# lh3/bfc

Hardware: AMD Instinct MI355X
Metric: M k-mers/s counted (bloom+htab) on 150 bp reads (higher is better)
Workload: dtype u64

## Files before the change

bfc_amd/csrc/bfcg_bloom3.hip:

```cpp
#include <hip/hip_runtime.h>
#include <stdint.h>
#include <stdlib.h>
#include "kmer_dev.h"
#include "bfcg_internal.h"
#include "bfcg_dev.h"

using namespace bfcg;

#define B3_UND 0x40000000u
#define B3_SEEN16 0x8000u
#define B3_COLD_NR 8
#define B3_WALK_U 4
template <int BT, int PF, bool COLD>
__global__ __launch_bounds__(BT, PF <= 2 ? 8 : 6) void k_bloom3(KParams P, BloomArgs A)
{
	extern __shared__ __attribute__((aligned(16))) unsigned char smem[];
	__shared__ uint32_t s_list_n, s_ovf, s_pool_off, s_emit_n, s_fs_used, s_wb_n, s_pad3[2];
	const uint32_t f = blockIdx.x;
	const bool ho_log = A.ho_stride != 0;
	if (batch_poisoned(A)) { if (ho_log && threadIdx.x == 0) A.ho_mark[f] = A.ho_cur[f]; return; }
	uint32_t rs, n;
	region_list(A, f, rs, n);
	if (n == 0) { if (threadIdx.x == 0) { if (ho_log) A.ho_mark[f] = A.ho_cur[f]; else if (A.agg_cnt) A.agg_cnt[f] = 0; } return; }
	uint32_t ho_cur0 = 0;
	unsigned long long *ho_base;
	if (ho_log) {
		ho_cur0 = A.ho_cur[f];
		if (ho_cur0 + n > A.ho_stride) {
			if (threadIdx.x == 0) { atomicAdd(&A.stats[(size_t)(f & (ST_SLOTS - 1)) * ST_N + ST_ERR_POOL], 1ULL); A.ho_mark[f] = ho_cur0; }
			return;
		}
		ho_base = A.ho + (uint64_t)f * A.ho_stride + ho_cur0;
	} else ho_base = reinterpret_cast<unsigned long long *>(A.stream_out) + rs;
	A.stats += (size_t)(f & (ST_SLOTS - 1)) * ST_N;
	const uint32_t region_dw = 16u << P.R;
	unsigned char *sp = smem;
	unsigned int *region = reinterpret_cast<unsigned int *>(sp); sp += (size_t)region_dw * 4;
	const uint32_t nblk = 1u << P.R;
	unsigned int *bcnt = reinterpret_cast<unsigned int *>(sp), *boff = bcnt + nblk;
	if (COLD) sp += (size_t)(2 * nblk + 4) * 4;
	unsigned int *fs = reinterpret_cast<unsigned int *>(sp); if (!COLD) sp += (size_t)P.fs_cap * 4;
	unsigned int *la = reinterpret_cast<unsigned int *>(sp); sp += (size_t)P.list_cap * 4;
	unsigned int *lb = reinterpret_cast<unsigned int *>(sp); sp += (size_t)P.list_cap * 4;
	unsigned short *lc = reinterpret_cast<unsigned short *>(sp); sp += (size_t)P.list_cap * 2;
	unsigned short *ord = reinterpret_cast<unsigned short *>(sp);
	const uint32_t fs_mask = P.fs_cap - 1;
	const uint32_t *recs = A.recs + (uint64_t)rs * 3;
	unsigned int *g_region = reinterpret_cast<unsigned int *>(A.bloom) + (uint64_t)f * region_dw;
	const uint32_t imp = (P.f_base + f) >> P.F2;
	const Dec3 D = dec3_geom(P);
	const int tid = threadIdx.x, lane = tid & 63;
	const uint32_t mask_a = (1u << D.a) - 1u, imp_sh = D.n ? imp << D.lo : 0u, sh_up = D.lo + D.n;
#ifdef BFCG_MEASURE
	const bool timing = BFCG_ABL(P, 64) && tid == 0;
	long long tq[7] = {0, 0, 0, 0, 0, 0, 0};
	long long tc[7] = {0, 0, 0, 0, 0, 0, 0};
	if (timing) tq[0] = clock64();
#define B3_TC(i) do { if (timing) tc[i] = clock64(); } while (0)
#else
#define B3_TC(i) do { } while (0)
#endif
	auto addr3 = [&](uint32_t d0, uint32_t d1) -> uint32_t {
		const uint32_t y0d = d0 & mask_a, upper = y0d >> D.up;
		const uint32_t y0lo = D.n ? (y0d & D.lowmask) | imp_sh | (upper << sh_up) : y0d;
		const uint32_t y1lo = __builtin_amdgcn_alignbit(d1, d0, D.a) & D.mk32;
		const uint32_t hh = upper | (((y0lo - y1lo) ^ y1lo) << D.sh_x);
		uint32_t h2 = (hh >> 9) & 511u;
		h2 |= (uint32_t)((h2 & 31u) == 0);
		return (y0d & D.rmask) | ((hh & 511u) << 8) | (h2 << 17);
	};
	auto entry3 = [&](uint32_t d0, uint32_t d1) -> unsigned long long {
		const unsigned long long AA = d0 | ((unsigned long long)d1 << 32);
		const unsigned long long y1 = (AA >> D.a) & ((1ULL << P.k) - 1);
		const uint32_t y0d = d0 & mask_a;
		const unsigned long long id = (unsigned long long)((y0d & D.rmask) | ((y0d >> D.up) << D.R)) | (y1 << D.sh_y1);
		return (id << 1) | (unsigned long long)((d1 >> D.sh_flag) & 1u);
	};
	RecW<3> cur[PF], nxt[PF];
#pragma unroll
	for (int u = 0; u < PF; ++u) {
		const uint32_t i = tid + u * BT;
		cur[u].d[0] = cur[u].d[1] = cur[u].d[2] = 0; nxt[u] = cur[u];
		if (i < n) cur[u] = rec_load<3>(recs + (uint64_t)i * 3);
		if (i + BT * PF < n) nxt[u] = rec_load<3>(recs + (uint64_t)(i + BT * PF) * 3);
	}
	{
		const uint4 *src = reinterpret_cast<const uint4 *>(g_region);
		uint4 *dst = reinterpret_cast<uint4 *>(region);
		for (uint32_t i = tid; i < region_dw / 4; i += BT) dst[i] = src[i];
		if constexpr (COLD) { for (uint32_t i = tid; i < 2 * nblk + 4; i += BT) bcnt[i] = 0; }
		else {
			uint4 *f4 = reinterpret_cast<uint4 *>(fs);
			for (uint32_t i = tid; i < P.fs_cap / 4; i += BT) f4[i] = make_uint4(FS32_EMPTY, FS32_EMPTY, FS32_EMPTY, FS32_EMPTY);
		}
		if (tid == 0) { s_list_n = 0; s_emit_n = 0; s_ovf = 0; s_fs_used = 0; s_wb_n = 0; }
	}
	__syncthreads();
#ifdef BFCG_MEASURE
	if (timing) tq[1] = clock64();
#endif
	volatile uint32_t *v_ovf = &s_ovf;

	for (uint32_t base = 0; base < n; base += BT * PF) {
		uint32_t pk[PF], um[PF];
#pragma unroll
		for (int u = 0; u < PF; ++u) {
			pk[u] = 0; um[u] = 0;
			if (base + u * BT + (uint32_t)(tid & ~63) < n) {
				pk[u] = addr3(cur[u].d[0], cur[u].d[1]);
				const B3Pos b = b3_positions((pk[u] >> 8) & 511u, pk[u] >> 17);
				const uint32_t bl64 = (pk[u] & 255u) << 6;
				const uint32_t w0 = *b3_wordp(region, bl64, b.b0), w1 = *b3_wordp(region, bl64, b.b1), w2 = *b3_wordp(region, bl64, b.b2), w3 = *b3_wordp(region, bl64, b.b3);
				um[u] = (b3_bit(w0, b.b0) | (b3_bit(w1, b.b1) << 1) | (b3_bit(w2, b.b2) << 2) | (b3_bit(w3, b.b3) << 3)) ^ 15u;
			}
		}
		unsigned long long ms[PF], ml[PF];
		uint32_t tot_s = 0, tot_l = 0;
#pragma unroll
		for (int u = 0; u < PF; ++u) {
			const bool act = base + tid + u * BT < n;
			ms[u] = __ballot(act && um[u] == 0); ml[u] = __ballot(act && um[u] != 0);
			tot_s += (uint32_t)__popcll(ms[u]); tot_l += (uint32_t)__popcll(ml[u]);
		}
		uint32_t o_s = 0, o_l = 0;
		if (lane == 0) { if (tot_s) o_s = atomicAdd(&s_emit_n, tot_s); if (tot_l) o_l = atomicAdd(&s_list_n, tot_l); }
		o_s = __builtin_amdgcn_readfirstlane(o_s); o_l = __builtin_amdgcn_readfirstlane(o_l);
#pragma unroll
		for (int u = 0; u < PF; ++u) {
			const uint32_t below_lo = (uint32_t)__builtin_amdgcn_mbcnt_lo((uint32_t)ms[u], 0u), below_s = (uint32_t)__builtin_amdgcn_mbcnt_hi((uint32_t)(ms[u] >> 32), below_lo);
			const uint32_t blow_lo = (uint32_t)__builtin_amdgcn_mbcnt_lo((uint32_t)ml[u], 0u), below_l = (uint32_t)__builtin_amdgcn_mbcnt_hi((uint32_t)(ml[u] >> 32), blow_lo);
			const bool act = base + tid + u * BT < n;
			if (act && um[u] == 0) {
				ho_base[o_s + below_s] = entry3(cur[u].d[0], cur[u].d[1]);
				if (A.seen_out) A.seen_out[cur[u].d[2]] = 2;
			} else if (act) {
				const uint32_t li = o_l + below_l;
				if (li < P.list_cap) {
					la[li] = cur[u].d[2]; lb[li] = pk[u] | (um[u] << 26); lc[li] = (unsigned short)(base + tid + u * BT);
					if constexpr (COLD) __hip_atomic_fetch_add(&bcnt[pk[u] & 255u], 1u, __ATOMIC_RELAXED, __HIP_MEMORY_SCOPE_WORKGROUP);
				}
			}
			o_s += (uint32_t)__popcll(ms[u]); o_l += (uint32_t)__popcll(ml[u]);
		}
		if (base + BT * PF < n) {
#pragma unroll
			for (int u = 0; u < PF; ++u) {
				cur[u] = nxt[u];
				const uint32_t i = base + 2 * BT * PF + tid + u * BT;
				if (i < n) nxt[u] = rec_load<3>(recs + (uint64_t)i * 3);
			}
		}
	}
	__syncthreads();
#ifdef BFCG_MEASURE
	if (timing) tq[2] = clock64();
#endif
	const uint32_t ln = s_list_n;
	const bool ovf_list = ln > P.list_cap || ln > (COLD ? (uint32_t)(B3_COLD_NR * BT) : 8191u) || n > 65535u;
	bool dirty = true;
	if constexpr (COLD) {
		if (!ovf_list) {
			B3_TC(0);
			if (tid < 64) {
				const uint32_t per = (nblk + 63u) >> 6, b0 = (uint32_t)tid * per;
				uint32_t v[4] = {0, 0, 0, 0}, sum = 0;
#pragma unroll
				for (int t = 0; t < 4; ++t) if ((uint32_t)t < per && b0 + t < nblk) { v[t] = bcnt[b0 + t]; sum += v[t]; }
				uint32_t inc = sum;
#pragma unroll
				for (int o = 1; o < 64; o <<= 1) { const uint32_t x = __shfl_up(inc, o); if (lane >= o) inc += x; }
				uint32_t run = inc - sum;
#pragma unroll
				for (int t = 0; t < 4; ++t) if ((uint32_t)t < per && b0 + t < nblk) { boff[b0 + t] = run; bcnt[b0 + t] = run; run += v[t]; }
				if (tid == 63) boff[nblk] = inc;
			}
			__syncthreads();
			B3_TC(1);
			uint32_t ex[B3_COLD_NR], ew[B3_COLD_NR], ep[B3_COLD_NR];
#pragma unroll
			for (int t = 0; t < B3_COLD_NR; ++t) {
				const uint32_t li = (uint32_t)tid + (uint32_t)t * BT;
				ex[t] = 0; ew[t] = 0; ep[t] = 0;
				if (li < ln) {
					ex[t] = la[li]; ew[t] = lb[li];
					ep[t] = ((uint32_t)lc[li] << 16) | __hip_atomic_fetch_add(&bcnt[ew[t] & 255u], 1u, __ATOMIC_RELAXED, __HIP_MEMORY_SCOPE_WORKGROUP);
				}
			}
			__syncthreads();
#pragma unroll
			for (int t = 0; t < B3_COLD_NR; ++t) {
				if ((uint32_t)tid + (uint32_t)t * BT < ln) { const uint32_t p = ep[t] & 0xffffu; la[p] = ex[t]; lb[p] = ew[t]; lc[p] = (unsigned short)(ep[t] >> 16); }
			}
			__syncthreads();
			B3_TC(2);
			uint32_t sx[B3_COLD_NR], sw[B3_COLD_NR], sq[B3_COLD_NR];
#pragma unroll
			for (int t = 0; t < B3_COLD_NR; ++t) {
				const uint32_t pos = (uint32_t)tid + (uint32_t)t * BT;
				sx[t] = 0; sw[t] = 0; sq[t] = 0;
				if (pos < ln) {
					const uint32_t x = la[pos], w = lb[pos], bl = w & 255u, s0 = boff[bl], s1 = boff[bl + 1], last = s1 - 1u;
					uint32_t r = s0;
					for (uint32_t j = s0; j < s1; j += 4) {
						const uint32_t y0 = la[j], y1 = la[min(j + 1u, last)], y2 = la[min(j + 2u, last)], y3 = la[min(j + 3u, last)];
						r += (uint32_t)(y0 < x) + (uint32_t)(j + 1u < s1 && y1 < x) + (uint32_t)(j + 2u < s1 && y2 < x) + (uint32_t)(j + 3u < s1 && y3 < x);
					}
					sx[t] = x; sw[t] = ((w >> 8) & 0x3ffffu) | (r << 18); sq[t] = lc[pos];
				}
			}
			__syncthreads();
			B3_TC(3);
#pragma unroll
			for (int t = 0; t < B3_COLD_NR; ++t) {
				if ((uint32_t)tid + (uint32_t)t * BT < ln) {
					const uint32_t r = sw[t] >> 18;
					const B3Pos b = b3_positions(sw[t] & 511u, (sw[t] >> 9) & 511u);
					la[r] = sx[t]; lb[r] = b.b0 | (b.b1 << 9) | (b.b2 << 18); ord[r] = (unsigned short)b.b3; lc[r] = (unsigned short)sq[t];
				}
			}
			__syncthreads();
			B3_TC(4);
			if ((uint32_t)tid < nblk) {
				const uint32_t bl = (uint32_t)tid, bl64 = bl << 6, s0 = boff[bl], s1 = boff[bl + 1], last = s1 - 1u;
				uint32_t pw_n[B3_WALK_U] = {0, 0, 0, 0}, p3_n[B3_WALK_U] = {0, 0, 0, 0};
				if (s0 < s1) {
#pragma unroll
					for (int u = 0; u < B3_WALK_U; ++u) { const uint32_t jj = min(s0 + (uint32_t)u, last); pw_n[u] = lb[jj]; p3_n[u] = ord[jj]; }
				}
				for (uint32_t j = s0; j < s1; j += B3_WALK_U) {
					uint32_t pw[B3_WALK_U], p3[B3_WALK_U], sn[B3_WALK_U];
#pragma unroll
					for (int u = 0; u < B3_WALK_U; ++u) { pw[u] = pw_n[u]; p3[u] = p3_n[u]; }
#pragma unroll
					for (int u = 0; u < B3_WALK_U; ++u) { const uint32_t jj = min(j + (uint32_t)(B3_WALK_U + u), last); pw_n[u] = lb[jj]; p3_n[u] = ord[jj]; }
#pragma unroll
					for (int u = 0; u < B3_WALK_U; ++u) {
						const uint32_t in = (uint32_t)(j + (uint32_t)u < s1);
						const uint32_t b0 = pw[u] & 511u, b1 = (pw[u] >> 9) & 511u, b2 = (pw[u] >> 18) & 511u, b3 = p3[u] & 511u;
						const uint32_t o0 = __hip_atomic_fetch_or(b3_wordp(region, bl64, b0), in << (b0 & 31u), __ATOMIC_RELAXED, __HIP_MEMORY_SCOPE_WORKGROUP);
						const uint32_t o1 = __hip_atomic_fetch_or(b3_wordp(region, bl64, b1), in << (b1 & 31u), __ATOMIC_RELAXED, __HIP_MEMORY_SCOPE_WORKGROUP);
						const uint32_t o2 = __hip_atomic_fetch_or(b3_wordp(region, bl64, b2), in << (b2 & 31u), __ATOMIC_RELAXED, __HIP_MEMORY_SCOPE_WORKGROUP);
						const uint32_t o3 = __hip_atomic_fetch_or(b3_wordp(region, bl64, b3), in << (b3 & 31u), __ATOMIC_RELAXED, __HIP_MEMORY_SCOPE_WORKGROUP);
						sn[u] = in & b3_bit(o0, b0) & b3_bit(o1, b1) & b3_bit(o2, b2) & b3_bit(o3, b3);
					}
#pragma unroll
					for (int u = 0; u < B3_WALK_U; ++u) if (sn[u]) ord[j + (uint32_t)u] = (unsigned short)(p3[u] | B3_SEEN16);
				}
			}
			__syncthreads();
			B3_TC(5);
			{
				uint32_t sm = 0, tot = 0;
#pragma unroll
				for (int t = 0; t < B3_COLD_NR; ++t) {
					const uint32_t li = (uint32_t)tid + (uint32_t)t * BT;
					if (li < ln) {
						const uint32_t seen = (ord[li] & B3_SEEN16) != 0;
						if (A.seen_out) A.seen_out[la[li]] = seen ? 2 : 1;
						sm |= seen << t;
					}
				}
#pragma unroll
				for (int t = 0; t < B3_COLD_NR; ++t) tot += (uint32_t)__popcll(__ballot((sm >> t) & 1u));
				if (tot) {
					uint32_t o = 0;
					if (lane == 0) o = atomicAdd(&s_emit_n, tot);
					o = __builtin_amdgcn_readfirstlane(o);
					RecW<3> r[B3_COLD_NR];
#pragma unroll
					for (int t = 0; t < B3_COLD_NR; ++t) {
						r[t].d[0] = r[t].d[1] = r[t].d[2] = 0;
						if ((sm >> t) & 1u) r[t] = rec_load<3>(recs + (uint64_t)lc[(uint32_t)tid + (uint32_t)t * BT] * 3);
					}
#pragma unroll
					for (int t = 0; t < B3_COLD_NR; ++t) {
						const unsigned long long vote = __ballot((sm >> t) & 1u);
						if ((sm >> t) & 1u) ho_base[o + (uint32_t)__builtin_amdgcn_mbcnt_hi((uint32_t)(vote >> 32), __builtin_amdgcn_mbcnt_lo((uint32_t)vote, 0u))] = entry3(r[t].d[0], r[t].d[1]);
						o += (uint32_t)__popcll(vote);
					}
				}
			}
			dirty = ln != 0;
			__syncthreads();
			B3_TC(6);
		}
	} else
	if (!ovf_list) {
		for (uint32_t li = tid; li < ln; li += BT) {
			const uint32_t w = lb[li], bl = w & 255u, bl64 = bl << 6, um = (w >> 26) & 15u;
			const B3Pos b = b3_positions((w >> 8) & 511u, (w >> 17) & 511u);
			uint32_t o0 = 0, o1 = 0, o2 = 0, o3 = 0;
			if (um & 1u) o0 = atomicOr(b3_wordp(region, bl64, b.b0), 1u << (b.b0 & 31u));
			if (um & 2u) o1 = atomicOr(b3_wordp(region, bl64, b.b1), 1u << (b.b1 & 31u));
			if (um & 4u) o2 = atomicOr(b3_wordp(region, bl64, b.b2), 1u << (b.b2 & 31u));
			if (um & 8u) o3 = atomicOr(b3_wordp(region, bl64, b.b3), 1u << (b.b3 & 31u));
			uint32_t cm = (b3_bit(o0, b.b0) | (b3_bit(o1, b.b1) << 1) | (b3_bit(o2, b.b2) << 2) | (b3_bit(o3, b.b3) << 3)) & um;
			if (cm) {
				*(volatile uint32_t *)&s_fs_used = 1;
				__hip_atomic_fetch_or(&region[bl * 16u], 1u, __ATOMIC_RELAXED, __HIP_MEMORY_SCOPE_WORKGROUP);
				const uint32_t idx = la[li];
				const uint32_t p01 = b.b0 | (b.b1 << 16), p23 = b.b2 | (b.b3 << 16);
				while (cm) {
					const int j = __ffs((int)cm) - 1;
					cm &= cm - 1;
					const uint32_t bj = ((j & 2 ? p23 : p01) >> ((j & 1) << 4)) & 0xffffu;
					if (!fs32_insert(fs, fs_mask, bl * 512u + bj, li, idx, la)) *v_ovf = 1;
				}
			}
		}
	}
	__syncthreads();
#ifdef BFCG_MEASURE
	if (timing) tq[6] = clock64();
#endif
	const bool ovf = ovf_list || s_ovf;
	if (COLD && !ovf) ;
	else if (!ovf) {
		if (s_fs_used) {
			auto compete_entry = [&](uint32_t li) {
				const uint32_t w = lb[li], bl = w & 255u, um = (w >> 26) & 15u;
				const B3Pos b = b3_positions((w >> 8) & 511u, (w >> 17) & 511u);
				const uint32_t q0 = bl * 512u + b.b0, q1 = bl * 512u + b.b1, q2 = bl * 512u + b.b2, q3 = bl * 512u + b.b3;
				const uint32_t c0 = fs[fs32_slot(q0, fs_mask)], c1 = fs[fs32_slot(q1, fs_mask)], c2 = fs[fs32_slot(q2, fs_mask)], c3 = fs[fs32_slot(q3, fs_mask)];
				uint32_t todo = ((uint32_t)(c0 != FS32_EMPTY) | ((uint32_t)(c1 != FS32_EMPTY) << 1) | ((uint32_t)(c2 != FS32_EMPTY) << 2) | ((uint32_t)(c3 != FS32_EMPTY) << 3)) & um;
				bool und = todo == um;
				if (todo) {
					const uint32_t idx = la[li];
					const uint32_t p01 = b.b0 | (b.b1 << 16), p23 = b.b2 | (b.b3 << 16);
					while (todo) {
						const int j = __ffs((int)todo) - 1;
						todo &= todo - 1;
						const uint32_t bj = ((j & 2 ? p23 : p01) >> ((j & 1) << 4)) & 0xffffu;
						und &= fs32_compete(fs, fs_mask, bl * 512u + bj, li, idx, la);
					}
				}
				if (und) lb[li] = w | B3_UND;
			};
			unsigned short *const wb = lc + ln;
			const uint32_t wb_cap = P.list_cap - ln;
			for (uint32_t li0 = 0; li0 < ln; li0 += BT) {
				const uint32_t li = li0 + tid;
				bool want = false;
				if (li < ln) {
					want = (region[(lb[li] & 255u) * 16u] & 1u) != 0;
					if (!want && A.seen_out) A.seen_out[la[li]] = 1;
				}
				const unsigned long long vote = __ballot(want);
				if (vote) {
					uint32_t o = 0;
					if (lane == 0) o = atomicAdd(&s_wb_n, (uint32_t)__popcll(vote));
					o = __builtin_amdgcn_readfirstlane(o);
					if (want) {
						const uint32_t slot = o + (uint32_t)__builtin_amdgcn_mbcnt_hi((uint32_t)(vote >> 32), __builtin_amdgcn_mbcnt_lo((uint32_t)vote, 0u));
						if (slot < wb_cap) wb[slot] = (unsigned short)li;
						else compete_entry(li);
					}
				}
			}
// ... 44 lines not shown
		uint64_t want = (uint64_t)n * nh * 2;
		const uint64_t lim = (uint64_t)(1u << P.R) * 512 * 2;
		if (want > lim) want = lim;
		uint32_t cap = 1024; while (cap < want) cap <<= 1;
		if (tid == 0) {
			uint32_t sl = f & (A.pool_slices - 1);
			while (atomicCAS(&A.pool[sl], 0ULL, 1ULL) != 0ULL) sl = (sl + 1) & (A.pool_slices - 1);
			s_pool_off = sl; s_emit_n = 0;
			atomicAdd(&A.stats[ST_SLOW_BUCKETS], 1ULL);
		}
		{
			const uint4 *src = reinterpret_cast<const uint4 *>(g_region);
			uint4 *dst = reinterpret_cast<uint4 *>(region);
			for (uint32_t i = tid; i < region_dw / 4; i += BT) dst[i] = src[i];
		}
		__syncthreads();
		unsigned long long *gfs = A.pool + A.pool_slices + (uint64_t)s_pool_off * lim;
		for (uint32_t i = tid; i < cap; i += BT) gfs[i] = FS_EMPTY;
		__threadfence();
		__syncthreads();
		const uint32_t gmask = cap - 1;
		for (uint32_t i = tid; i < n; i += BT) {
			const RecW<3> r = rec_load<3>(recs + (uint64_t)i * 3);
			const uint32_t w = addr3(r.d[0], r.d[1]), bl = w & 255u;
			uint32_t z = (w >> 8) & 511u;
			for (int j = 0; j < nh; ++j) {
				const uint32_t b = bloom_next(z, w >> 17);
				if (!b3_bit(*b3_wordp(region, bl << 6, b), b)) fs_insert<true>(gfs, gmask, bl * 512 + b, r.d[2], gmask);
			}
		}
		__threadfence();
		__syncthreads();
		for (uint32_t i0 = 0; i0 < n; i0 += BT) {
			const uint32_t i = i0 + tid;
			bool seen = false;
			RecW<3> r; r.d[0] = r.d[1] = r.d[2] = 0;
			if (i < n) {
				r = rec_load<3>(recs + (uint64_t)i * 3);
				const uint32_t w = addr3(r.d[0], r.d[1]), bl = w & 255u;
				uint32_t z = (w >> 8) & 511u; bool first = false, unresolved = false;
				for (int j = 0; j < nh; ++j) {
					uint32_t b = bloom_next(z, w >> 17), fi;
					if (fs_lookup<true>(gfs, gmask, bl * 512 + b, fi)) {
						unresolved = true; first |= (fi == r.d[2]);
						atomicOr(b3_wordp(region, bl << 6, b), 1u << (b & 31));
					}
				}
				seen = !unresolved || !first;
				if (A.seen_out) A.seen_out[r.d[2]] = seen ? 2 : 1;
			}
			const unsigned long long vote = __ballot(seen);
			if (vote) {
				uint32_t o = 0;
				if (lane == 0) o = atomicAdd(&s_emit_n, (uint32_t)__popcll(vote));
				o = __builtin_amdgcn_readfirstlane(o);
				if (seen) ho_base[o + (uint32_t)__popcll(vote & ((1ULL << lane) - 1))] = entry3(r.d[0], r.d[1]);
			}
		}
		__syncthreads();
		if (tid == 0) { __threadfence(); atomicExch(&A.pool[s_pool_off], 0ULL); }
	}
#ifdef BFCG_MEASURE
	if (timing) tq[3] = clock64();
#endif
	if (dirty) {
		uint4 *dst = reinterpret_cast<uint4 *>(g_region);
		const uint4 *src = reinterpret_cast<const uint4 *>(region);
		for (uint32_t i = tid; i < region_dw / 4; i += BT) dst[i] = src[i];
	}
#ifdef BFCG_MEASURE
	if (timing) tq[4] = clock64();
#endif
	if (tid == 0) {
		const uint32_t ns = s_emit_n;
		if (ns) atomicAdd(&A.stats[ST_SEEN], (unsigned long long)ns);
		if (ho_log) { A.ho_cur[f] = ho_cur0 + ns; A.ho_mark[f] = ho_cur0 + ns; }
		else if (A.agg_cnt) A.agg_cnt[f] = ns;
	}
#ifdef BFCG_MEASURE
	if (timing) {
		tq[5] = clock64();
		if (BFCG_ABL(P, 128)) {
			if (COLD) for (int t = 0; t < 6; ++t) atomicAdd(&A.stats[10 + t], (unsigned long long)(tc[t + 1] - tc[t]));
		} else {
			for (int t = 0; t < 5; ++t) atomicAdd(&A.stats[10 + t], (unsigned long long)(tq[t + 1] - tq[t]));
			atomicAdd(&A.stats[15], (unsigned long long)(tq[6] - tq[2]));
		}
	}
#endif
#undef B3_TC
	(void)s_pad3;
}

namespace bfcg {

typedef void (*BloomFn)(KParams, BloomArgs);
static BloomFn bloom3_kernel(bool pf2, bool cold)
{
	if (cold) return pf2 ? k_bloom3<512, 2, true> : k_bloom3<512, 4, true>;
	return pf2 ? k_bloom3<512, 2, false> : k_bloom3<512, 4, false>;
}
static hipError_t set_bloom3_max_lds(BloomFn fn, int lds) { return hipFuncSetAttribute((const void *)fn, hipFuncAttributeMaxDynamicSharedMemorySize, lds < BLOOM3_LDS_FLOOR ? BLOOM3_LDS_FLOOR : lds); }
hipError_t set_bloom3_lds_attr(int lds)
{
	hipError_t e = hipSuccess;
	for (int i = 0; i < 4 && e == hipSuccess; ++i) e = set_bloom3_max_lds(bloom3_kernel(i & 1, i & 2), lds);
	return e;
}

void run_bloom3(const KParams &P, const BloomArgs &A, int nfine, size_t lds, hipStream_t st)
{
	static int pf = 0;
	if (!pf) { const char *e = getenv("BFCG_B3_PF"); pf = e && atoi(e) == 2 ? 2 : e && atoi(e) == 4 ? 4 : 1; }
	const bool pf2 = P.b3_cold ? P.b3_warm != 0 : pf == 2 || (pf == 1 && P.b3_warm);
	hipLaunchKernelGGL(bloom3_kernel(pf2, P.b3_cold != 0), dim3(nfine), dim3(512), lds, st, P, A);
}

}

struct Dec4 { int up, iw, is; uint32_t rmask; };
__device__ __forceinline__ Dec4 dec4_geom(const KParams &P)
{
	Dec4 g;
	g.up = P.rec_n ? P.rec_lo : P.bf_shift - 9;
	const int io = (P.k - P.rec_n) + P.k + 1;
	g.iw = io >> 5; g.is = io & 31; g.rmask = (1u << P.R) - 1u;
	return g;
}
template <int BT, int PF>
__global__ __launch_bounds__(BT, 6) void k_bloom3fm(KParams P, BloomArgs A)
{
	extern __shared__ __attribute__((aligned(16))) unsigned char smem[];
	__shared__ uint32_t s_list_n, s_seen;
	const uint32_t f = blockIdx.x;
	if (batch_poisoned(A)) return;
	uint32_t rs, n;
	region_list(A, f, rs, n);
	if (n == 0) return;
	A.stats += (size_t)(f & (ST_SLOTS - 1)) * ST_N;
	const uint32_t region_dw = 16u << P.R, nblk = 1u << P.R;
	unsigned char *sp = smem;
	unsigned int *region = reinterpret_cast<unsigned int *>(sp); sp += (size_t)region_dw * 4;
	unsigned int *region_hi = reinterpret_cast<unsigned int *>(sp); sp += (size_t)region_dw * 4;
	unsigned int *bcnt = reinterpret_cast<unsigned int *>(sp), *boff = bcnt + nblk; sp += (size_t)(2 * nblk + 4) * 4;
	unsigned int *la = reinterpret_cast<unsigned int *>(sp); sp += (size_t)P.list_cap * 4;
	unsigned int *lb = reinterpret_cast<unsigned int *>(sp); sp += (size_t)P.list_cap * 4;
	unsigned short *ord = reinterpret_cast<unsigned short *>(sp);
	const uint32_t *recs = A.recs + (uint64_t)rs * 4;
	unsigned int *g_region = reinterpret_cast<unsigned int *>(A.bloom) + (uint64_t)f * region_dw;
	unsigned int *g_region_hi = reinterpret_cast<unsigned int *>(A.bloom_hi) + (uint64_t)f * region_dw;
	const Dec4 D = dec4_geom(P);
	const int tid = threadIdx.x, lane = tid & 63;
	auto addr4 = [&](uint32_t d0, uint32_t d1) -> uint32_t {
		const uint32_t hh = __builtin_amdgcn_alignbit(d1, d0, D.up);
		uint32_t h2 = (hh >> 9) & 511u;
		h2 |= (uint32_t)((h2 & 31u) == 0);
		return (d0 & D.rmask) | ((hh & 511u) << 8) | (h2 << 17);
	};
	auto idx4 = [&](const RecW<4> &r) -> uint32_t {
		const uint32_t a = D.iw == 0 ? r.d[0] : D.iw == 1 ? r.d[1] : D.iw == 2 ? r.d[2] : r.d[3], b = D.iw == 0 ? r.d[1] : D.iw == 1 ? r.d[2] : r.d[3];
		return D.is ? __builtin_amdgcn_alignbit(b, a, D.is) : a;
	};
	auto set_hi = [&](uint32_t bl64, const B3Pos &b) {
		__hip_atomic_fetch_or(b3_wordp(region_hi, bl64, b.b0), 1u << (b.b0 & 31u), __ATOMIC_RELAXED, __HIP_MEMORY_SCOPE_WORKGROUP);
		__hip_atomic_fetch_or(b3_wordp(region_hi, bl64, b.b1), 1u << (b.b1 & 31u), __ATOMIC_RELAXED, __HIP_MEMORY_SCOPE_WORKGROUP);
		__hip_atomic_fetch_or(b3_wordp(region_hi, bl64, b.b2), 1u << (b.b2 & 31u), __ATOMIC_RELAXED, __HIP_MEMORY_SCOPE_WORKGROUP);
		__hip_atomic_fetch_or(b3_wordp(region_hi, bl64, b.b3), 1u << (b.b3 & 31u), __ATOMIC_RELAXED, __HIP_MEMORY_SCOPE_WORKGROUP);
	};
	{
		const uint4 *src = reinterpret_cast<const uint4 *>(g_region), *src2 = reinterpret_cast<const uint4 *>(g_region_hi);
		uint4 *dst = reinterpret_cast<uint4 *>(region), *dst2 = reinterpret_cast<uint4 *>(region_hi);
		for (uint32_t i = tid; i < region_dw / 4; i += BT) { dst[i] = src[i]; dst2[i] = src2[i]; }
	}
	uint32_t r = 0, sh = 32, seen_total = 0;
	bool dirty = false;
	const uint32_t cap = P.list_cap < (uint32_t)(B3_COLD_NR * BT) ? P.list_cap : (uint32_t)(B3_COLD_NR * BT);
	for (;;) {
		for (uint32_t i = tid; i < 2 * nblk + 4; i += BT) bcnt[i] = 0;
		if (tid == 0) { s_list_n = 0; s_seen = 0; }
		__syncthreads();
		uint32_t my_seen = 0;
		RecW<4> rec[PF], nxt[PF];
#pragma unroll
		for (int u = 0; u < PF; ++u) {
			const uint32_t i = tid + u * BT;
			rec[u].d[0] = rec[u].d[1] = rec[u].d[2] = rec[u].d[3] = 0; nxt[u] = rec[u];
			if (i < n) rec[u] = rec_load<4>(recs + (uint64_t)i * 4);
			if (i + BT * PF < n) nxt[u] = rec_load<4>(recs + (uint64_t)(i + BT * PF) * 4);
		}
		for (uint32_t base = 0; base < n; base += BT * PF) {
			uint32_t pk[PF], um[PF], ix[PF];
			bool act[PF];
#pragma unroll
			for (int u = 0; u < PF; ++u) {
				ix[u] = idx4(rec[u]);
				act[u] = base + tid + u * BT < n && (sh == 32 || (ix[u] >> sh) == r);
				pk[u] = addr4(rec[u].d[0], rec[u].d[1]);
				const B3Pos b = b3_positions((pk[u] >> 8) & 511u, pk[u] >> 17);
// ... 132 lines not shown
```

bfc_amd/csrc/bfcg_ctx.hip:

```cpp
#include <hip/hip_runtime.h>
#include <stdint.h>
#include <stdio.h>
#include <stdlib.h>
#include <string.h>
#include <stdarg.h>
#include <sys/mman.h>
#include <time.h>
#include <vector>
#include <thread>
#include "bfc_gpu.h"
#include "bfcg_internal.h"
#include "bfc_host.h"

using namespace bfcg;

static thread_local char g_err[512] = "";
enum { HO_MAX_PAGES = BFCG_HO_MAX_PAGES };
enum { OP_FLAG_WORDS = 12, OP_STICKY = 8 };
static double dbg_now(void) { struct timespec ts; clock_gettime(CLOCK_MONOTONIC, &ts); return ts.tv_sec + 1e-9 * ts.tv_nsec; }
static inline void set_seg_shift(KParams &P, int s, int blk_max) { P.seg_shift = s; P.seg_blk = s < blk_max ? s : blk_max; }
int bfcg::fail(const char *fmt, ...)
{
	va_list ap; va_start(ap, fmt); vsnprintf(g_err, sizeof(g_err), fmt, ap); va_end(ap);
	fprintf(stderr, "[E::bfcg] %s\n", g_err);
// ... 121 lines not shown
	P.k = prm->k; P.q = prm->q; P.bf_shift = prm->bf_shift; P.n_hashes = prm->n_hashes; P.filter_mode = prm->filter_mode;
	P.l_pre = clamp_lpre(prm->k, prm->l_pre);
	if (!prm->filter_mode && 2 * prm->k < P.l_pre) {
		fail("k=%d is too small for l_pre=%d: the count table needs 2k >= l_pre (htab.c:45-58)", prm->k, P.l_pre); bfcg_destroy(c); return NULL;
	}
	{
		const char *e;
		P.R = prm->region_shift > 0 ? prm->region_shift : ((e = getenv("BFCG_R")) ? atoi(e) : 8);
		if (P.R > 10) P.R = 10;
		if (P.R < 4) P.R = 4;
		if (P.R > P.bf_shift - 9) P.R = P.bf_shift - 9;
		while (P.bf_shift - 9 - P.R > 20 && P.R < 10) ++P.R;
		P.F = P.bf_shift - 9 - P.R;
		if (P.F <= 8) { P.F1 = P.F; P.F2 = 0; }
		else { P.F2 = (P.F + 1) / 2; if (P.F2 > 10) P.F2 = 10; P.F1 = P.F - P.F2; }
		if (P.F2 > 0 && (e = getenv("BFCG_F1"))) {
			const int f1 = atoi(e);
			if (f1 >= 1 && f1 <= 10 && P.F - f1 >= 1 && P.F - f1 <= 10 && f1 >= log2n) { P.F1 = f1; P.F2 = P.F - f1; }
		}
		if (P.F1 > 10) { fail("bf_shift=%d needs more than two scatter levels at region_shift=%d", P.bf_shift, P.R); bfcg_destroy(c); return NULL; }
		if (n_ranks > 1 && P.F2 == 0) {
			if (P.F <= log2n) { fail("bf_shift=%d gives %d bloom regions: too few for %d ranks", P.bf_shift, 1 << P.F, n_ranks); bfcg_destroy(c); return NULL; }
			P.F1 = (P.F + 1) / 2 > log2n ? (P.F + 1) / 2 : log2n; P.F2 = P.F - P.F1;
		}
#ifdef BFCG_MEASURE
		P.ablate = (e = getenv("BFCG_ABLATE")) ? atoi(e) : 0;
#else
		P.ablate = 0;
		if ((e = getenv("BFCG_ABLATE")) && atoi(e)) fprintf(stderr, "[W::bfcg] BFCG_ABLATE=%s ignored: this library was built without -DBFCG_MEASURE\n", e);
#endif
		{ const char *e = getenv("BFCG_REC_DROP"); P.rec_n = (P.k >= P.bf_shift - 9 && bfcg_rec_dwords(P.k, P.F1) < bfcg_rec_dwords(P.k, 0) && !(e && atoi(e) == 0)) ? P.F1 : 0; P.rec_lo = P.R + P.F2; }
		c->rw = 4 * bfcg_rec_dwords(P.k, P.rec_n);
		P.ag_cap = (e = getenv("BFCG_AG")) ? (uint32_t)atoi(e) : 256;
		const size_t region = (size_t)64 << P.R;
		size_t rwb = 8;
		{
			const char *es = getenv("BFCG_SEG");
			P.seg_lo = P.R < P.k ? P.R : P.k;
			P.seg_hi = P.k < P.bf_shift - 9 ? P.k : P.bf_shift - 9;
			if (P.seg_hi < P.seg_lo) P.seg_hi = P.seg_lo;
			const int id_bits = 2 * P.k - (P.seg_hi - P.seg_lo);
			c->seg_ok = !prm->filter_mode && !prm->track_order && P.R <= 8 && !getenv("BFCG_BT") && id_bits <= BFC_CH_KEYBITS && prm->table_layout != 1 && !(es && atoi(es) == 0);
			P.seg = c->seg_ok;
			c->b3_ok = c->seg_ok && prm->n_hashes == 4 && c->rw == 12 && bloom3_geometry_ok(P) && !getenv("BFCG_NO_B3");
			P.b3 = c->b3_ok;
			if (P.b3) rwb = 10;
		}
		const size_t second = prm->filter_mode ? region : P.seg ? 0 : (size_t)P.ag_cap * ((P.k > 32 ? 24 : 16) + (prm->track_order ? 8 : 0));
		size_t budget = (size_t)53000;
		if (region + second + 16 * 1024 > budget) budget = 80 * 1024 - 1024;
		if (region + second + 16 * 1024 > budget) budget = 160 * 1024 - 1024;
		if ((e = getenv("BFCG_LDS")) != 0 && (size_t)atoi(e) >= region + second + 4096 && (size_t)atoi(e) <= 160 * 1024 - 1024) budget = (size_t)atoi(e);
		size_t left = budget - region - second - 16;
		uint32_t fs = 512, best_fs = 512, best_list = 0;
		for (; fs <= 32768 && (size_t)fs * 4 + rwb * 64 <= left; fs <<= 1) {
			uint32_t list = (uint32_t)((left - (size_t)fs * 4) / rwb);
			if (list > fs / 4 * 3) list = fs / 4 * 3;
			if (list > best_list) { best_list = list; best_fs = fs; }
		}
		fs = best_fs;
		if ((e = getenv("BFCG_FS")) != 0) { fs = (uint32_t)atoi(e); best_list = (uint32_t)((left - (size_t)fs * 4) / rwb); }
		P.fs_cap = fs;
		P.list_cap = best_list;
		if (P.list_cap > 8191) P.list_cap = 8191;
		c->fs_cap_w = c->list_cap_w = 0;
		if (P.b3 && !getenv("BFCG_LDS") && !(getenv("BFCG_B3_WARM") && atoi(getenv("BFCG_B3_WARM")) == 0)) {
			const size_t bw = 40900;
			if (bw > region + 16 + 8192) {
				const size_t lw = bw - region - 16;
				uint32_t fw = fs; while (fw > 1024 && (size_t)fw * 4 + (size_t)(P.list_cap / 4 * 3) * rwb > lw) fw >>= 1;
				uint32_t l = (size_t)fw * 4 < lw ? (uint32_t)((lw - (size_t)fw * 4) / rwb) : 0;
				if (l > P.list_cap) l = P.list_cap;
				if (l >= P.list_cap / 4 * 3 && fw >= 1024) { c->fs_cap_w = fw; c->list_cap_w = l; }
			}
		}
		c->list_cap_c = 0; c->list_cap_cw = 0;
		if (P.b3 && !(getenv("BFCG_B3_COLD") && atoi(getenv("BFCG_B3_COLD")) == 0)) {
			const size_t fixed = region + ((size_t)2 << P.R) * 4 + 16 + 16;
			if (budget > fixed + 12 * 256) {
				uint32_t l = (uint32_t)((budget - fixed) / 12);
				if (l > 4096) l = 4096;
				c->list_cap_c = l;
			}
			c->list_cap_cw = 0;
			if ((size_t)40900 > fixed + 12 * 256 && getenv("BFCG_B3_WALK_WARM") && atoi(getenv("BFCG_B3_WALK_WARM"))) c->list_cap_cw = (uint32_t)(((size_t)40900 - fixed) / 12);
		}
		P.b3fm = 0;
		if (prm->filter_mode && c->rw == 16 && bloom3fm_geometry_ok(P) && !getenv("BFCG_NO_B3")) {
			const size_t fixed = 2 * region + ((size_t)2 << P.R) * 4 + 16 + 16;
			if (budget > fixed + 10 * 256) {
				uint32_t l = (uint32_t)((budget - fixed) / 10);
				if ((e = getenv("BFCG_B3FM_LIST")) != 0 && atoi(e) >= 64 && (uint32_t)atoi(e) < l) l = (uint32_t)atoi(e);
				if (l > 4096) l = 4096;
				P.b3fm = 1; P.list_cap = l; P.fs_cap = 512;
			}
		}
		{
			const size_t room = (size_t)P.fs_cap * 4 + (size_t)P.list_cap * 8;
			uint32_t ct = 1; while ((size_t)ct * 2 * 8 <= room) ct <<= 1;
			P.ct_cap = ct;
		}
	}
	P.tab_cshift = prm->tab_cshift > 0 ? prm->tab_cshift : (P.l_pre <= 20 ? 5 : 3);
	if (prm->tab_cshift <= 0)
		while ((1ULL << (P.l_pre + P.tab_cshift)) < prm->max_batch_pos / 4 && P.l_pre + P.tab_cshift < 34) ++P.tab_cshift;
	P.track = (prm->track_order && !prm->filter_mode) ? 1 : 0;
	{ const char *e = getenv("BFCG_BT"); P.bloom_bt = e ? atoi(e) : (bloom_lds_bytes(P) > 80 * 1024 && !P.track && P.n_hashes == 4) ? 1024 : 512; if (P.bloom_bt != 1024 || P.track || P.n_hashes != 4) P.bloom_bt = 512; }
	c->n_ranks = n_ranks; c->rank = prm->rank; c->log2n = log2n;
	{ const char *e = getenv("BFCG_PIPELINE"); c->pipeline = e ? atoi(e) != 0 : prm->max_batch_pos <= (1ULL << 28); }

	if (n_ranks > 1 && log2n > P.F1) { fail("multi-GPU needs a two-level partition with 2^F1=%d >= n_ranks (bf_shift=%d is too small)", 1 << P.F1, P.bf_shift); bfcg_destroy(c); return NULL; }
	P.idx_rank = n_ranks > 1 ? (uint32_t)prm->rank << (32 - log2n) : 0u;
	c->bloom_bytes = (1ULL << (P.bf_shift - 3)) >> log2n;

	BatchBufs &B = c->B;
	B.max_kmers = prm->max_batch_pos;
	const int nb1 = 1 << P.F1, nfine = (1 << P.F) >> log2n;
	c->recv_cap = n_ranks > 1 ? B.max_kmers + B.max_kmers / 4 + (1u << 20) : B.max_kmers;
	BFCG_CKN(bfcg_destroy(c), hipStreamCreate(&c->st)); BFCG_CKN(bfcg_destroy(c), hipStreamCreate(&c->stA)); BFCG_CKN(bfcg_destroy(c), hipStreamCreate(&c->stC));
	for (int b = 0; b < 2; ++b) {
		for (int i = 0; i < 7; ++i) BFCG_CKN(bfcg_destroy(c), hipEventCreate(&c->evt[b][i]));
		BFCG_CKN(bfcg_destroy(c), hipEventCreateWithFlags(&c->evA[b], hipEventDisableTiming)); BFCG_CKN(bfcg_destroy(c), hipEventCreateWithFlags(&c->evB[b], hipEventDisableTiming));
	}
	BFCG_CKN(bfcg_destroy(c), hipEventCreateWithFlags(&c->evCopy, hipEventDisableTiming));
	{
		const uint64_t tile = (uint64_t)bfcg_tile_of_rw(c->rw / 4), tile1 = (uint64_t)bfcg_tile1_of_rw(c->rw / 4);
		const uint64_t tiles1 = (prm->max_batch_pos + tile1 - 1) / tile1, chunks1 = (tiles1 + BFCG_SCAN_CH - 1) / BFCG_SCAN_CH;
		const uint64_t rows2 = (c->recv_cap + c->recv_cap / 8) / tile + (uint64_t)nb1 * 16 + 8;
		for (int b = 0; b < 2; ++b) {
			BFCG_CKN(bfcg_destroy(c), hipMalloc(&c->rows1[b], sizeof(uint32_t) * tiles1 * nb1));
			BFCG_CKN(bfcg_destroy(c), hipMalloc(&c->chunk1[b], sizeof(uint32_t) * chunks1 * nb1));
			BFCG_CKN(bfcg_destroy(c), hipMalloc(&c->start1[b], sizeof(uint32_t) * (nb1 + 1) * 2));
		}
		B.rows1 = c->rows1[0]; B.chunk1 = c->chunk1[0]; B.start1 = c->start1[0]; B.row_base = B.start1 + nb1 + 1;
		if (P.F2 > 0) {
			BFCG_CKN(bfcg_destroy(c), hipMalloc(&B.rows2, sizeof(uint32_t) * rows2 * (1u << P.F2)));
			BFCG_CKN(bfcg_destroy(c), hipMalloc(&B.start2, sizeof(uint32_t) * (nfine + 1)));
		}
	}
	{
		const char *e = getenv("BFCG_ONEPASS");
		c->onepass_ok = n_ranks == 1 && P.F2 > 0 && !(e && atoi(e) == 0);
		uint64_t cap = (B.max_kmers + B.max_kmers / 8) / ((uint64_t)nb1 * 8) + 1;
		while (cap * nb1 * 8 > 0xffffffffULL) --cap;
		if (cap >= 1024) cap &= ~31ULL;
		else if (cap >= 8) cap &= ~3ULL;
		c->op_cap = (uint32_t)cap;
		c->op_min_pos = (e = getenv("BFCG_ONEPASS_MIN_TILES")) ? (uint64_t)atoi(e) * 4096 : (uint64_t)nb1 * 8 * 1024;
	}
	const uint64_t recs1_n = c->onepass_ok ? (uint64_t)c->op_cap * nb1 * 8 + (uint64_t)bfcg_tile1_of_rw(c->rw / 4) + 64 : B.max_kmers;
	BFCG_CKN(bfcg_destroy(c), hipMalloc(&c->recs1[0], recs1_n * c->rw));
	if (n_ranks == 1 && !c->pipeline) c->recs1[1] = c->recs1[0];
	else BFCG_CKN(bfcg_destroy(c), hipMalloc(&c->recs1[1], recs1_n * c->rw));
	{
		const char *e = getenv("BFCG_ONEPASS");
		c->mg_op2_ok = P.F2 > 0 && !(e && atoi(e) == 0);
	}
	{ const char *e = getenv("BFCG_MG_SLABS"); c->mg_slab_ok = P.F2 > 0 && !(e && atoi(e) == 0); }
	if (c->onepass_ok || c->mg_slab_ok) {
		for (int b = 0; b < 2; ++b) {
			BFCG_CKN(bfcg_destroy(c), hipMalloc(&c->op_cursor[b], sizeof(uint32_t) * (8 * nb1 * 32 + 32)));
			BFCG_CKN(bfcg_destroy(c), hipMalloc(&c->op_seg[b], sizeof(uint32_t) * ((size_t)25 * nb1 + 8)));
		}
	}
	if (c->mg_slab_ok) for (int b = 0; b < 2; ++b) BFCG_CKN(bfcg_destroy(c), hipHostMalloc(&c->h_rows[b], sizeof(uint32_t) * ((size_t)8 * nb1 + 2 * (size_t)n_ranks)));
	if (c->onepass_ok || c->mg_op2_ok || c->mg_slab_ok) {
		for (int b = 0; b < 2; ++b) BFCG_CKN(bfcg_destroy(c), hipHostMalloc(&c->h_flags[b], 4 * sizeof(uint32_t)));
		BFCG_CKN(bfcg_destroy(c), hipMalloc(&c->op_flags, OP_FLAG_WORDS * sizeof(uint32_t)));
// ... 1249 lines not shown
```

Before: 41410.

## Enable warm cold-walk bloom3 variant by default with smaller per-thread list arrays

Adds an NR template parameter so the cold/walk bloom3 kernel can use 4 list slots per thread instead of 8 when the list capacity fits. This cuts register arrays in the sort and walk phases. It also simplifies the COLD-path miss test to a single AND-reduced bit, since the per-hash miss mask is no longer stored. The warm walk variant (list_cap_cw) is now on by default rather than opt-in. This changes which kernel runs on the warm path and trades a smaller LDS list for lower register pressure and possibly higher occupancy.

```diff
diff --git a/bfc_amd/csrc/bfcg_bloom3.hip b/bfc_amd/csrc/bfcg_bloom3.hip
--- a/bfc_amd/csrc/bfcg_bloom3.hip
+++ b/bfc_amd/csrc/bfcg_bloom3.hip
@@ -10,8 +10,9 @@
 #define B3_UND 0x40000000u
 #define B3_SEEN16 0x8000u
 #define B3_COLD_NR 8
+#define B3_WARM_NR 4
 #define B3_WALK_U 4
-template <int BT, int PF, bool COLD>
+template <int BT, int PF, bool COLD, int NR>
 __global__ __launch_bounds__(BT, PF <= 2 ? 8 : 6) void k_bloom3(KParams P, BloomArgs A)
 {
 	extern __shared__ __attribute__((aligned(16))) unsigned char smem[];
@@ -111,7 +112,8 @@
 				const B3Pos b = b3_positions((pk[u] >> 8) & 511u, pk[u] >> 17);
 				const uint32_t bl64 = (pk[u] & 255u) << 6;
 				const uint32_t w0 = *b3_wordp(region, bl64, b.b0), w1 = *b3_wordp(region, bl64, b.b1), w2 = *b3_wordp(region, bl64, b.b2), w3 = *b3_wordp(region, bl64, b.b3);
-				um[u] = (b3_bit(w0, b.b0) | (b3_bit(w1, b.b1) << 1) | (b3_bit(w2, b.b2) << 2) | (b3_bit(w3, b.b3) << 3)) ^ 15u;
+				if constexpr (COLD) um[u] = (((w0 >> (b.b0 & 31u)) & (w1 >> (b.b1 & 31u)) & (w2 >> (b.b2 & 31u)) & (w3 >> (b.b3 & 31u))) & 1u) ^ 1u;
+				else um[u] = (b3_bit(w0, b.b0) | (b3_bit(w1, b.b1) << 1) | (b3_bit(w2, b.b2) << 2) | (b3_bit(w3, b.b3) << 3)) ^ 15u;
 			}
 		}
 		unsigned long long ms[PF], ml[PF];
@@ -136,7 +138,7 @@
 			} else if (act) {
 				const uint32_t li = o_l + below_l;
 				if (li < P.list_cap) {
-					la[li] = cur[u].d[2]; lb[li] = pk[u] | (um[u] << 26); lc[li] = (unsigned short)(base + tid + u * BT);
+					la[li] = cur[u].d[2]; lb[li] = COLD ? pk[u] : pk[u] | (um[u] << 26); lc[li] = (unsigned short)(base + tid + u * BT);
 					if constexpr (COLD) __hip_atomic_fetch_add(&bcnt[pk[u] & 255u], 1u, __ATOMIC_RELAXED, __HIP_MEMORY_SCOPE_WORKGROUP);
 				}
 			}
@@ -156,7 +158,7 @@
 	if (timing) tq[2] = clock64();
 #endif
 	const uint32_t ln = s_list_n;
-	const bool ovf_list = ln > P.list_cap || ln > (COLD ? (uint32_t)(B3_COLD_NR * BT) : 8191u) || n > 65535u;
+	const bool ovf_list = ln > P.list_cap || ln > (COLD ? (uint32_t)(NR * BT) : 8191u) || n > 65535u;
 	bool dirty = true;
 	if constexpr (COLD) {
 		if (!ovf_list) {
@@ -176,9 +178,9 @@
 			}
 			__syncthreads();
 			B3_TC(1);
-			uint32_t ex[B3_COLD_NR], ew[B3_COLD_NR], ep[B3_COLD_NR];
-#pragma unroll
-			for (int t = 0; t < B3_COLD_NR; ++t) {
+			uint32_t ex[NR], ew[NR], ep[NR];
+#pragma unroll
+			for (int t = 0; t < NR; ++t) {
 				const uint32_t li = (uint32_t)tid + (uint32_t)t * BT;
 				ex[t] = 0; ew[t] = 0; ep[t] = 0;
 				if (li < ln) {
@@ -188,14 +190,14 @@
 			}
 			__syncthreads();
 #pragma unroll
-			for (int t = 0; t < B3_COLD_NR; ++t) {
+			for (int t = 0; t < NR; ++t) {
 				if ((uint32_t)tid + (uint32_t)t * BT < ln) { const uint32_t p = ep[t] & 0xffffu; la[p] = ex[t]; lb[p] = ew[t]; lc[p] = (unsigned short)(ep[t] >> 16); }
 			}
 			__syncthreads();
 			B3_TC(2);
-			uint32_t sx[B3_COLD_NR], sw[B3_COLD_NR], sq[B3_COLD_NR];
-#pragma unroll
-			for (int t = 0; t < B3_COLD_NR; ++t) {
+			uint32_t sx[NR], sw[NR], sq[NR];
+#pragma unroll
+			for (int t = 0; t < NR; ++t) {
 				const uint32_t pos = (uint32_t)tid + (uint32_t)t * BT;
 				sx[t] = 0; sw[t] = 0; sq[t] = 0;
 				if (pos < ln) {
@@ -211,7 +213,7 @@
 			__syncthreads();
 			B3_TC(3);
 #pragma unroll
-			for (int t = 0; t < B3_COLD_NR; ++t) {
+			for (int t = 0; t < NR; ++t) {
 				if ((uint32_t)tid + (uint32_t)t * BT < ln) {
 					const uint32_t r = sw[t] >> 18;
 					const B3Pos b = b3_positions(sw[t] & 511u, (sw[t] >> 9) & 511u);
@@ -252,7 +254,7 @@
 			{
 				uint32_t sm = 0, tot = 0;
 #pragma unroll
-				for (int t = 0; t < B3_COLD_NR; ++t) {
+				for (int t = 0; t < NR; ++t) {
 					const uint32_t li = (uint32_t)tid + (uint32_t)t * BT;
 					if (li < ln) {
 						const uint32_t seen = (ord[li] & B3_SEEN16) != 0;
@@ -261,19 +263,19 @@
 					}
 				}
 #pragma unroll
-				for (int t = 0; t < B3_COLD_NR; ++t) tot += (uint32_t)__popcll(__ballot((sm >> t) & 1u));
+				for (int t = 0; t < NR; ++t) tot += (uint32_t)__popcll(__ballot((sm >> t) & 1u));
 				if (tot) {
 					uint32_t o = 0;
 					if (lane == 0) o = atomicAdd(&s_emit_n, tot);
 					o = __builtin_amdgcn_readfirstlane(o);
-					RecW<3> r[B3_COLD_NR];
-#pragma unroll
-					for (int t = 0; t < B3_COLD_NR; ++t) {
+					RecW<3> r[NR];
+#pragma unroll
+					for (int t = 0; t < NR; ++t) {
 						r[t].d[0] = r[t].d[1] = r[t].d[2] = 0;
 						if ((sm >> t) & 1u) r[t] = rec_load<3>(recs + (uint64_t)lc[(uint32_t)tid + (uint32_t)t * BT] * 3);
 					}
 #pragma unroll
-					for (int t = 0; t < B3_COLD_NR; ++t) {
+					for (int t = 0; t < NR; ++t) {
 						const unsigned long long vote = __ballot((sm >> t) & 1u);
 						if ((sm >> t) & 1u) ho_base[o + (uint32_t)__builtin_amdgcn_mbcnt_hi((uint32_t)(vote >> 32), __builtin_amdgcn_mbcnt_lo((uint32_t)vote, 0u))] = entry3(r[t].d[0], r[t].d[1]);
 						o += (uint32_t)__popcll(vote);
@@ -484,6 +486,10 @@
 		tq[5] = clock64();
 		if (BFCG_ABL(P, 128)) {
 			if (COLD) for (int t = 0; t < 6; ++t) atomicAdd(&A.stats[10 + t], (unsigned long long)(tc[t + 1] - tc[t]));
+			else if (!ovf) {
+				atomicAdd(&A.stats[13], (unsigned long long)(tq[6] - tq[2]));
+				atomicAdd(&A.stats[14], (unsigned long long)(tq[3] - tq[6]));
+			}
 		} else {
 			for (int t = 0; t < 5; ++t) atomicAdd(&A.stats[10 + t], (unsigned long long)(tq[t + 1] - tq[t]));
 			atomicAdd(&A.stats[15], (unsigned long long)(tq[6] - tq[2]));
@@ -497,16 +503,16 @@
 namespace bfcg {
 
 typedef void (*BloomFn)(KParams, BloomArgs);
-static BloomFn bloom3_kernel(bool pf2, bool cold)
+static BloomFn bloom3_kernel(bool pf2, bool cold, bool nr4)
 {
-	if (cold) return pf2 ? k_bloom3<512, 2, true> : k_bloom3<512, 4, true>;
-	return pf2 ? k_bloom3<512, 2, false> : k_bloom3<512, 4, false>;
+	if (cold) return !pf2 ? k_bloom3<512, 4, true, B3_COLD_NR> : nr4 ? k_bloom3<512, 2, true, B3_WARM_NR> : k_bloom3<512, 2, true, B3_COLD_NR>;
+	return pf2 ? k_bloom3<512, 2, false, 0> : k_bloom3<512, 4, false, 0>;
 }
 static hipError_t set_bloom3_max_lds(BloomFn fn, int lds) { return hipFuncSetAttribute((const void *)fn, hipFuncAttributeMaxDynamicSharedMemorySize, lds < BLOOM3_LDS_FLOOR ? BLOOM3_LDS_FLOOR : lds); }
 hipError_t set_bloom3_lds_attr(int lds)
 {
 	hipError_t e = hipSuccess;
-	for (int i = 0; i < 4 && e == hipSuccess; ++i) e = set_bloom3_max_lds(bloom3_kernel(i & 1, i & 2), lds);
+	for (int i = 0; i < 8 && e == hipSuccess; ++i) e = set_bloom3_max_lds(bloom3_kernel(i & 1, i & 2, i & 4), lds);
 	return e;
 }
 
@@ -515,7 +521,8 @@
 	static int pf = 0;
 	if (!pf) { const char *e = getenv("BFCG_B3_PF"); pf = e && atoi(e) == 2 ? 2 : e && atoi(e) == 4 ? 4 : 1; }
 	const bool pf2 = P.b3_cold ? P.b3_warm != 0 : pf == 2 || (pf == 1 && P.b3_warm);
-	hipLaunchKernelGGL(bloom3_kernel(pf2, P.b3_cold != 0), dim3(nfine), dim3(512), lds, st, P, A);
+	const bool nr4 = P.list_cap <= (uint32_t)(B3_WARM_NR * 512);
+	hipLaunchKernelGGL(bloom3_kernel(pf2, P.b3_cold != 0, nr4), dim3(nfine), dim3(512), lds, st, P, A);
 }
 
 }
diff --git a/bfc_amd/csrc/bfcg_ctx.hip b/bfc_amd/csrc/bfcg_ctx.hip
--- a/bfc_amd/csrc/bfcg_ctx.hip
+++ b/bfc_amd/csrc/bfcg_ctx.hip
@@ -227,8 +227,7 @@
 				if (l > 4096) l = 4096;
 				c->list_cap_c = l;
 			}
-			c->list_cap_cw = 0;
-			if ((size_t)40900 > fixed + 12 * 256 && getenv("BFCG_B3_WALK_WARM") && atoi(getenv("BFCG_B3_WALK_WARM"))) c->list_cap_cw = (uint32_t)(((size_t)40900 - fixed) / 12);
+			if ((size_t)40900 > fixed + 12 * 256 && !(getenv("BFCG_B3_WALK_WARM") && atoi(getenv("BFCG_B3_WALK_WARM")) == 0)) c->list_cap_cw = (uint32_t)(((size_t)40900 - fixed) / 12);
 		}
 		P.b3fm = 0;
 		if (prm->filter_mode && c->rw == 16 && bloom3fm_geometry_ok(P) && !getenv("BFCG_NO_B3")) {
```

Result: faster. 42090 (median of 6 runs) (+1.6%).
